# LBM-EPFL/MaD

Measured on AMD Instinct MI355X. Metric: anchor-pair x rotation correlations/sec on 256^3 map; top-k pose agreement, higher is better.
Workload: dtype i8 (correlation, exact int32 accumulate) / f64 (binning, pose scoring)

## Files before the change

### mad_amd/csrc/mad_common.h

```cpp
#pragma once

#include <hip/hip_runtime.h>

#include <cmath>
#include <cstdarg>
#include <cstdint>
#include <cstdio>
#include <cstdlib>
#include <cstring>

#include "../../include/mad_amd.h"

#define MAD_WAVE 64
#define MAD_ZLUT 1024
#define MAD_MAX_BELT 32


struct __attribute__((aligned(16))) EqspFastLds {
    float g32[MAD_MAX_Z][4];
    float z_in_lo[MAD_MAX_BELT], z_in_hi[MAD_MAX_BELT], belt_lo0[MAD_MAX_BELT], belt_inv_w[MAD_MAX_BELT];
    int belt_first[MAD_MAX_BELT], belt_count[MAD_MAX_BELT];
    unsigned char zlut[MAD_ZLUT];
    float4 belt_f[MAD_MAX_BELT];
    int2 belt_i[MAD_MAX_BELT];
// ... 19 lines not shown

struct EqspDev {
    int Z;
    int nbelt;
    double th_lo[MAD_MAX_Z];
    double th_hi[MAD_MAX_Z];
    double ph_lo[MAD_MAX_Z];
    double ph_hi[MAD_MAX_Z];
    int belt_first[MAD_MAX_Z];
    int belt_count[MAD_MAX_Z];
    double to_dom[MAD_MAX_Z][9];
    double adj_sec[MAD_MAX_Z][9];
    unsigned char zlut[MAD_ZLUT];
    float z_in_lo[MAD_MAX_BELT];
    float z_in_hi[MAD_MAX_BELT];
    float belt_lo0[MAD_MAX_BELT];
    float belt_inv_w[MAD_MAX_BELT];
    int belt_first32[MAD_MAX_BELT];
    int belt_count32[MAD_MAX_BELT];
    float g32[MAD_MAX_Z][4];
    EqspFastLds image;
    EqspTabLds tab;
    int tab_ok;
};

#ifndef MAD_EQSP_GUARD
#define MAD_EQSP_GUARD 4e-5
#endif

struct FieldDev {
    const float4 *tex;
    int nx, ny, nz;
    const unsigned *tex4;
};


struct DevBuf {
    void *p = nullptr;
    size_t cap = 0;
};

enum { MAD_T_ORIENT = 0, MAD_T_DESCRIBE, MAD_T_CORRELATE, MAD_T_PAIRS, MAD_T_POSE, MAD_T_TOPK, MAD_T_REFINE,
       MAD_T_DENSITY, MAD_T_CCC, MAD_T_SEG_PARENT, MAD_T_SEG_JUMP, MAD_T_SEG_SCAN, MAD_T_SEG_SMOOTH, MAD_T_COUNT };

#define MAD_T_RING 32
#define MAD_LANES 8
#define MAD_BRACKETS 3
#define MAD_SHARD_RING 8
#define MAD_DIST_BUFS 6
#define MAD_RES (2 * MAD_LANES)

struct TimerGroup {
    hipEvent_t start[MAD_T_RING];
    hipEvent_t stop[MAD_T_RING];
    int pending = 0;
    double total_ms = 0.0;
    int64_t launches = 0;
};

struct DensityDev {
    float *grid = nullptr;
    float4 *grad = nullptr;
    int nx = 0, ny = 0, nz = 0;
    double o[3] = {0, 0, 0};
    double vs = 0;
};
// ... 358 lines not shown
        if (i + 2 * T < n4) d4[i + 2 * T] = v2;
        if (i + 3 * T < n4) d4[i + 3 * T] = v3;
    }
    const int tail = (int)((bytes & 15) >> 2);
    if ((int)threadIdx.x < tail) ((unsigned *)lds_dst)[4 * n4 + threadIdx.x] = ((const unsigned *)src)[4 * n4 + threadIdx.x];
}

__device__ __forceinline__ int cvt_floor(float x) {
    int r;
    asm("v_cvt_flr_i32_f32 %0, %1" : "=v"(r) : "v"(x));
    return r;
}
__device__ __forceinline__ unsigned mad_u24(unsigned a, unsigned b, unsigned c) {
    unsigned r;
    asm("v_mad_u32_u24 %0, %1, %2, %3" : "=v"(r) : "v"(a), "v"(b), "v"(c));
    return r;
}
__device__ __forceinline__ int cvt_round(float x) {
    int r;
    asm("v_cvt_rpi_i32_f32 %0, %1" : "=v"(r) : "v"(x));
    return r;
}

__device__ __forceinline__ void eqsp_fast_stage(const EqspDev *t, EqspFastLds *l) { stage_lds(l, &t->image, sizeof(EqspFastLds)); }

__device__ __forceinline__ unsigned mad_tex4_encode(float x, float y, float z, float w) {
    if (!(fabsf(x) <= 3.0e38f) || !(fabsf(y) <= 3.0e38f) || !(fabsf(z) <= 3.0e38f) || !(w <= 3.0e38f)) return 0x80000000u;
    if (w < 1e-5f) return 0xC0000000u;
    const float inv = 511.0f / w;
    const int ix = min(max((int)rintf(x * inv), -511), 511), iy = min(max((int)rintf(y * inv), -511), 511), iz = min(max((int)rintf(z * inv), -511), 511);
    return ((unsigned)ix & 0x3ffu) | (((unsigned)iy & 0x3ffu) << 10) | (((unsigned)iz & 0x3ffu) << 20);
}

__device__ __forceinline__ int eqsp_tab32(const EqspTabLds *t, float x, float y, float z) {
    const int bz = min(max(cvt_floor(fmaf(z, 0.5f * MAD_TAB_ZBINS, 0.5f * MAD_TAB_ZBINS)), 0), MAD_TAB_ZBINS - 1);
    const int b = t->zbelt[bz];
    const float xr = x * __builtin_amdgcn_rcpf(fmaxf(fabsf(x) + fabsf(y), 1e-30f));
    const float u = copysignf(fmaf(xr, 0.25f * MAD_TAB_PBINS, 0.25f * MAD_TAB_PBINS), y);
    const int bp = min(max(cvt_floor(0.5f * MAD_TAB_PBINS - u), 0), MAD_TAB_PBINS - 1);
    const int zn = t->ptab[b & (MAD_TAB_BELTS - 1)][bp];
    return (b | zn) >= 255 ? -1 : zn;
}

template <class F>
__device__ __forceinline__ void eqsp_classify_lds(const EqspFastLds *t, double th, double sth, double ph, F &&f) {
    const int nb = t->nbelt;
    for (int b = 0; b < nb; b++) {
        if (ph < t->ph_hi[b] && ph > t->ph_lo[b]) {
            const int a0 = t->belt_first[b], a1 = a0 + t->belt_count[b];
            for (int a = a0; a < a1; a++) {
                const double lo = t->th_lo[a], hi = t->th_hi[a];
                if ((th < hi && th > lo) || (sth < hi && sth > lo)) f(a);
            }
            break;
        }
    }
}

__device__ __forceinline__ float approx_angle(float x, float y) {
    const float ax = fabsf(x), ay = fabsf(y);
    const float mx = fmaxf(ax, ay), mn = fminf(ax, ay);
    const float q = mn * __builtin_amdgcn_rcpf(fmaxf(mx, 1e-30f));
    const float q2 = q * q;
    float a = fmaf(q2, -0.011769974f, 0.052822195f);
    a = fmaf(q2, a, -0.116649978f);
    a = fmaf(q2, a, 0.193669885f);
// ... 78 lines not shown
```

### mad_amd/csrc/mad_ctx.hip

```cpp
#include "mad_common.h"

static char g_init_err[512] = "";
#define MAD_TWO_PI_H 6.283185307179586476925286766559

int mad_fail(mad_ctx *ctx, int code, const char *fmt, ...) {
    char *dst = ctx ? ctx->err : g_init_err;
    va_list ap;
    va_start(ap, fmt);
    vsnprintf(dst, 512, fmt, ap);
    va_end(ap);
    return code;
}

extern "C" const char *mad_last_error(const mad_ctx *ctx) { return ctx ? ctx->err : g_init_err; }

int mad_reserve(mad_ctx *ctx, DevBuf &b, size_t bytes) {
    if (bytes == 0) bytes = 16;
    if (b.cap >= bytes) return MAD_OK;
    if (b.p) {
        MAD_HIP(hipStreamSynchronize(ctx->stream));
        (void)hipFree(b.p);
        b.p = nullptr;
        b.cap = 0;
    }
// ... 305 lines not shown
        for (int a = 0; a < MAD_MAX_Z; a++) { im.th_lo[a] = h.th_lo[a]; im.th_hi[a] = h.th_hi[a]; }
        im.nbelt = h.nbelt;
        im.tier2_ok = getenv("MAD_NO_TIER2") ? 0 : 1;
        for (int a = 0; a < Z; a++) {
            im.dir[a][0] = cos(h.th_lo[a]); im.dir[a][1] = sin(h.th_lo[a]);
            im.dir[a][2] = cos(h.th_hi[a]); im.dir[a][3] = sin(h.th_hi[a]);
        }
        for (int b = 0; b < h.nbelt; b++) {
            const double m[2] = {MAD_T2_MARGIN64, MAD_T2_MARGIN32};
            for (int k = 0; k < 2; k++) {
                im.zthr[b][2 * k] = h.ph_lo[b] <= 0.0 ? 2.0 : cos(h.ph_lo[b] + m[k]);
                im.zthr[b][2 * k + 1] = h.ph_hi[b] - m[k] >= 3.14159265358979323846 ? -2.0 : cos(h.ph_hi[b] - m[k]);
            }
            if (h.belt_count[b] > 1)
                for (int a = h.belt_first[b]; a < h.belt_first[b] + h.belt_count[b]; a++)
                    if (!(h.th_hi[a] - h.th_lo[a] < 3.0) || !(h.th_hi[a] > h.th_lo[a])) im.tier2_ok = 0;
            if (b + 1 < h.nbelt && h.ph_hi[b] != h.ph_lo[b + 1]) im.tier2_ok = 0;
        }
    }
    {
        static const bool no_tab = getenv("MAD_NO_TAB") != nullptr;
        h.tab_ok = mad_eqsp_tab_build(bounds, Z, h.tab.zbelt, &h.tab.ptab[0][0]) == 1 && !no_tab ? 1 : 0;
    }
    if (to_dom) memcpy(h.to_dom, to_dom, sizeof(double) * 9 * Z);
    if (adj_sec) memcpy(h.adj_sec, adj_sec, sizeof(double) * 9 * Z);
    MAD_HIP(hipMemcpyAsync(ctx->eq[which], &h, sizeof(EqspDev), hipMemcpyHostToDevice, ctx->stream));
    MAD_HIP(hipStreamSynchronize(ctx->stream));
    ctx->eq_set[which] = true;
    return MAD_OK;
}


__global__ __launch_bounds__(256) void k_pack_field(const float *__restrict__ gx, const float *__restrict__ gy,
                                                    const float *__restrict__ gz, float4 *__restrict__ tex, unsigned *__restrict__ tex4, size_t n) {
    size_t i = (size_t)blockIdx.x * blockDim.x + threadIdx.x;
    const size_t step = (size_t)gridDim.x * blockDim.x;
    for (; i < n; i += step) {
        const float x = gx[i], y = gy[i], z = gz[i];
        const float s = __fadd_rn(__fadd_rn(__fmul_rn(x, x), __fmul_rn(y, y)), __fmul_rn(z, z));
        const float w = sqrtf(s);
        tex[i] = make_float4(x, y, z, w);
        tex4[i] = mad_tex4_encode(x, y, z, w);
    }
}

int mad_field_alloc(mad_ctx *ctx, int slot, int nx, int ny, int nz, size_t *n_out) {
    if (slot < 0 || slot >= MAD_MAX_FIELDS) return mad_fail(ctx, MAD_EINVAL, "field slot %d out of range", slot);
    if (nx < 2 || ny < 2 || nz < 2) return mad_fail(ctx, MAD_EINVAL, "field dims %dx%dx%d", nx, ny, nz);
    const size_t n = (size_t)nx * ny * nz;
    if (n >= ((size_t)1 << 32) || (size_t)nx * ny >= ((size_t)1 << 24) || nz >= (1 << 24))
        return mad_fail(ctx, MAD_EINVAL, "field of %dx%dx%d texels: more than 2^32 texels or 2^24 per x-y plane", nx, ny, nz);
    if (ctx->field_mem[slot]) {
        MAD_HIP(hipStreamSynchronize(ctx->stream));
        (void)hipFree(ctx->field_mem[slot]);
        ctx->field_mem[slot] = nullptr;
        ctx->fields[slot] = FieldDev{nullptr, 0, 0, 0};
    }
    hipError_t e = hipMalloc(&ctx->field_mem[slot], n * (sizeof(float4) + sizeof(unsigned)));
    if (e != hipSuccess) {
        ctx->field_mem[slot] = nullptr;
        return mad_fail(ctx, MAD_ENOMEM, "field of %zu texels: %s", n, hipGetErrorString(e));
    }
    ctx->fields[slot] = FieldDev{(const float4 *)ctx->field_mem[slot], nx, ny, nz, (const unsigned *)((const float4 *)ctx->field_mem[slot] + n)};
    *n_out = n;
    return MAD_OK;
}

extern "C" int mad_upload_field_device(mad_ctx *ctx, int slot, const float *g3, int nx, int ny, int nz) {
    if (!ctx || !g3) return MAD_EINVAL;
    size_t n = 0;
    MAD_TRY(mad_field_alloc(ctx, slot, nx, ny, nz, &n));
    const int blocks = (int)std::min<size_t>(mad_ceil_div((int64_t)n, 256), (size_t)ctx->n_cu * 16);
    hipLaunchKernelGGL(k_pack_field, dim3(blocks), dim3(256), 0, ctx->stream, g3, g3 + n, g3 + 2 * n,
                       (float4 *)ctx->field_mem[slot], (unsigned *)((float4 *)ctx->field_mem[slot] + n), n);
    MAD_HIP(hipGetLastError());
    MAD_HIP(hipStreamSynchronize(ctx->stream));
    return MAD_OK;
}

extern "C" int mad_upload_field(mad_ctx *ctx, int slot, const float *gx, const float *gy, const float *gz, int nx,
                                int ny, int nz) {
    if (!ctx || !gx || !gy || !gz) return MAD_EINVAL;
    const size_t n = (size_t)nx * ny * nz;
    float *stage = nullptr;
    hipError_t e = hipMalloc((void **)&stage, 3 * n * sizeof(float));
    if (e != hipSuccess) return mad_fail(ctx, MAD_ENOMEM, "field staging: %s", hipGetErrorString(e));
    int rc = MAD_OK;
    if (hipMemcpyAsync(stage, gx, n * sizeof(float), hipMemcpyHostToDevice, ctx->stream) != hipSuccess ||
        hipMemcpyAsync(stage + n, gy, n * sizeof(float), hipMemcpyHostToDevice, ctx->stream) != hipSuccess ||
        hipMemcpyAsync(stage + 2 * n, gz, n * sizeof(float), hipMemcpyHostToDevice, ctx->stream) != hipSuccess)
        rc = mad_fail(ctx, MAD_EHIP, "field upload failed");
    if (rc == MAD_OK) rc = mad_upload_field_device(ctx, slot, stage, nx, ny, nz);
    (void)hipStreamSynchronize(ctx->stream);
    (void)hipFree(stage);
    return rc;
}

extern "C" int mad_free_field(mad_ctx *ctx, int slot) {
    if (!ctx || slot < 0 || slot >= MAD_MAX_FIELDS) return MAD_EINVAL;
    if (ctx->field_mem[slot]) {
        MAD_HIP(hipStreamSynchronize(ctx->stream));
        (void)hipFree(ctx->field_mem[slot]);
    }
    ctx->field_mem[slot] = nullptr;
    ctx->fields[slot] = FieldDev{nullptr, 0, 0, 0};
    return MAD_OK;
}

extern "C" int mad_field_download(mad_ctx *ctx, int slot, float *tex_xyzw, uint32_t *tex4) {
    if (!ctx) return MAD_EINVAL;
    if (slot < 0 || slot >= MAD_MAX_FIELDS || !ctx->field_mem[slot]) return mad_fail(ctx, MAD_EINVAL, "mad_field_download: slot %d is empty or out of range", slot);
    const FieldDev &f = ctx->fields[slot];
    const size_t n = (size_t)f.nx * f.ny * f.nz;
    MAD_HIP(hipStreamSynchronize(ctx->stream));
    if (tex_xyzw) MAD_HIP(hipMemcpyAsync(tex_xyzw, f.tex, n * sizeof(float4), hipMemcpyDeviceToHost, ctx->stream));
    if (tex4) MAD_HIP(hipMemcpyAsync(tex4, f.tex4, n * sizeof(unsigned), hipMemcpyDeviceToHost, ctx->stream));
    MAD_HIP(hipStreamSynchronize(ctx->stream));
    return MAD_OK;
}


__global__ __launch_bounds__(256) void k_zero_words(uint4 *__restrict__ p, size_t n16) {
    for (size_t i = (size_t)blockIdx.x * blockDim.x + threadIdx.x; i < n16; i += (size_t)gridDim.x * blockDim.x) p[i] = make_uint4(0, 0, 0, 0);
}

__global__ __launch_bounds__(256) void k_copy_words(uint4 *__restrict__ dst, const uint4 *__restrict__ src, size_t n16) {
    for (size_t i = (size_t)blockIdx.x * blockDim.x + threadIdx.x; i < n16; i += (size_t)gridDim.x * blockDim.x) dst[i] = src[i];
}

void mad_zero_words(mad_ctx *ctx, void *p, size_t bytes) {
    const size_t n16 = (bytes + 15) / 16;
    hipLaunchKernelGGL(k_zero_words, dim3((unsigned)std::min<size_t>((n16 + 255) / 256, 1024)), dim3(256), 0, ctx->stream, (uint4 *)p, n16);
}

__global__ __launch_bounds__(256) void k_zero_words3(uint4 *__restrict__ p, size_t n16, uint4 *__restrict__ q, size_t m16, uint4 *__restrict__ r,
                                                     size_t l16) {
    for (size_t i = (size_t)blockIdx.x * blockDim.x + threadIdx.x; i < n16 + m16 + l16; i += (size_t)gridDim.x * blockDim.x) {
        if (i < n16) p[i] = make_uint4(0, 0, 0, 0);
        else if (i < n16 + m16) q[i - n16] = make_uint4(0, 0, 0, 0);
        else r[i - n16 - m16] = make_uint4(0, 0, 0, 0);
    }
}

void mad_zero_words3(mad_ctx *ctx, void *p, size_t bytes_p, void *q, size_t bytes_q, void *r, size_t bytes_r) {
    const size_t n16 = (bytes_p + 15) / 16, m16 = (bytes_q + 15) / 16, l16 = (bytes_r + 15) / 16;
    hipLaunchKernelGGL(k_zero_words3, dim3((unsigned)std::min<size_t>((n16 + m16 + l16 + 255) / 256, 1024)), dim3(256), 0, ctx->stream, (uint4 *)p,
                       n16, (uint4 *)q, m16, (uint4 *)r, l16);
}

void mad_copy_words(mad_ctx *ctx, void *dst, const void *src, size_t bytes) {
// ... 194 lines not shown
```

### mad_amd/csrc/mad_orient.hip

```cpp
#include <type_traits>

#include "mad_common.h"

#ifndef ORI_THREADS
#define ORI_THREADS 512
#endif
#define ORI_MAX_FAN 64
#define ORI_QUEUE 512
#define ORI_MAX_MAIN 8


static int ensure_mask(mad_ctx *ctx, int r) {
    if (ctx->mask_r == r) return MAD_OK;
    const int B = 2 * r + 1;
    int8_t *h = (int8_t *)malloc((size_t)B * B * B * 4);
    int n = 0;
    for (int i = -r; i <= r; i++)
        for (int j = -r; j <= r; j++)
            for (int k = -r; k <= r; k++)
                if (sqrt((double)(i * i + j * j + k * k)) <= r * 1.05) {
                    h[4 * n] = (int8_t)i; h[4 * n + 1] = (int8_t)j; h[4 * n + 2] = (int8_t)k; h[4 * n + 3] = 0;
                    n++;
                }
    if (ctx->mask_off) {
// ... 716 lines not shown
    const EqspDev *eq;
    int16_t *dsc;
    int8_t *dsc8;
    double *norm;
    int32_t *rsum;
};

__device__ __forceinline__ int describe_exact(const EqspFastLds *eq, float4 t, const double *R) {
    float gx = t.x, gy = t.y, gz = t.z;
    if (t.w > 1e-12f) { gx = __fdiv_rn(gx, t.w); gy = __fdiv_rn(gy, t.w); gz = __fdiv_rn(gz, t.w); }
    const double g0 = gx, g1 = gy, g2 = gz;
    const double rx = g0 * R[0] + g1 * R[1] + g2 * R[2];
    const double ry = g0 * R[3] + g1 * R[4] + g2 * R[5];
    const double rz = g0 * R[6] + g1 * R[7] + g2 * R[8];
    int zone = 0;
    classify_exact64(eq, eq, rx, ry, rz, [&](int zn) { zone = zn; });
    return zone;
}

__device__ __forceinline__ bool lattice_voxel_exact(double l0, double l1, double l2, const double *inv, double c0, double c1, double c2,
                                                    const FieldDev &F, int *v0, int *v1, int *v2) {
    const double p0 = (l0 * inv[0] + l1 * inv[1] + l2 * inv[2]) + c0;
    const double p1 = (l0 * inv[3] + l1 * inv[4] + l2 * inv[5]) + c1;
    const double p2 = (l0 * inv[6] + l1 * inv[7] + l2 * inv[8]) + c2;
    if (!(p0 >= 0.0) || !(p0 <= (double)(F.nx - 1)) || !(p1 >= 0.0) || !(p1 <= (double)(F.ny - 1)) || !(p2 >= 0.0) ||
        !(p2 <= (double)(F.nz - 1)))
        return false;
    int a0i = min((int)floor(p0), F.nx - 2), a1i = min((int)floor(p1), F.ny - 2), a2i = min((int)floor(p2), F.nz - 2);
    *v0 = (p0 - (double)a0i <= 0.5) ? a0i : a0i + 1;
    *v1 = (p1 - (double)a1i <= 0.5) ? a1i : a1i + 1;
    *v2 = (p2 - (double)a2i <= 0.5) ? a2i : a2i + 1;
    return true;
}
__device__ __forceinline__ unsigned lattice_index_exact(double l0, double l1, double l2, const double *inv, double c0, double c1, double c2,
                                                        const FieldDev &F, bool *oob) {
    int a0i, a1i, a2i;
    if (!lattice_voxel_exact(l0, l1, l2, inv, c0, c1, c2, F, &a0i, &a1i, &a2i)) {
        *oob = true;
        return 0;
    }
    return (unsigned)(((size_t)a0i * F.ny + a1i) * F.nz + a2i);
}

template <int S, int NSUB> __device__ __forceinline__ int sub_blk(int x) {
    if (NSUB == 64) return x / (S / 4);
    if (NSUB == 27) return x < S / 3 ? 0 : (x < 2 * S / 3 ? 1 : 2);
    if (NSUB == 8) return x < S / 2 ? 0 : 1;
    return 0;
}
template <int S, int NSUB> __device__ __forceinline__ int sub_of_jk(int j, int k) {
    if (NSUB == 64) return sub_blk<S, NSUB>(j) * 16 + sub_blk<S, NSUB>(k);
    if (NSUB == 27) return sub_blk<S, NSUB>(j) * 9 + sub_blk<S, NSUB>(k);
    if (NSUB == 8) return sub_blk<S, NSUB>(j) * 2 + (1 - sub_blk<S, NSUB>(k));
    return 0;
}
template <int S, int NSUB> __device__ __forceinline__ int sub_of_i(int i) {
    if (NSUB == 64) return sub_blk<S, NSUB>(i) * 4;
    if (NSUB == 27) return sub_blk<S, NSUB>(i) * 3;
    if (NSUB == 8) return sub_blk<S, NSUB>(i) * 4;
    return 0;
}

#define DSC_CHUNK 8
#ifndef DSC_PASSES
#define DSC_PASSES 1
#endif
#ifndef DSC_OCC
#define DSC_OCC 4
#endif
#define DSC_QUEUE_TAB 768
#ifdef MAD_PROBE_STAMPS
__device__ long long dsc_stamps[16384 * 8];
__device__ int dsc_open[16384];
// ... 60 lines not shown
    const int D = NSUB * Z;
    for (int i = tid; i < D; i += NT) hist[i] = 0;
    const int32_t *const p_perm = A.row_perm, *const p_anchor = A.row_anchor, *const p_coords = A.anc_coords, *const p_octave = A.anc_octave;
    const double *const p_R = A.row_R, *const p_Rinv = A.row_Rinv;
    const int uni_octave = A.uniform_octave;
    auto chain_record = [=](int64_t w, int *rec) {
        const int r = p_perm ? p_perm[w] : (int)w;
        const int an = p_anchor ? p_anchor[r] : r;
        rec[0] = r;
        rec[1] = p_coords[3 * an]; rec[2] = p_coords[3 * an + 1]; rec[3] = p_coords[3 * an + 2];
        rec[4] = p_octave ? p_octave[an] : uni_octave;
        double *inv = (double *)(rec + 8);
        if (p_Rinv) {
            for (int i = 0; i < 9; i++) inv[i] = p_Rinv[9 * (int64_t)r + i];
        } else {
            double m[9];
            mad_mat3_inv(p_R + 9 * (int64_t)r, m);
            for (int i = 0; i < 9; i++) inv[i] = m[i];
        }
    };
    const int *const recs = (const int *)A.row_rec;
    if (recs) {
        if (tid < 32) s_rec[tid] = recs[work * MAD_ROWREC_WORDS + tid];
    } else if (tid == 0) chain_record(work, s_rec);
    if (tid == 0) { s_oob = 0; s_nq = 0; }
    __syncthreads();
    const int64_t row = __builtin_amdgcn_readfirstlane(s_rec[0]);
    const int oct = __builtin_amdgcn_readfirstlane(s_rec[4]);
    const double *const sInv = (const double *)&s_rec[8];
    FieldDev F;
    F.tex = oct == 1 ? F1.tex : F0.tex; F.nx = oct == 1 ? F1.nx : F0.nx; F.ny = oct == 1 ? F1.ny : F0.ny; F.nz = oct == 1 ? F1.nz : F0.nz;
    F.tex4 = oct == 1 ? F1.tex4 : F0.tex4;
#ifdef DSC_TEX_AUX
    const __amdgpu_buffer_rsrc_t tex_rsrc = __builtin_amdgcn_make_buffer_rsrc((void *)F.tex4, 0, F.nx * F.ny * F.nz * 4, 0x00020000);
#define DSC_TEX4(at) ((unsigned)__builtin_amdgcn_raw_buffer_load_b32(tex_rsrc, (int)((at) * 4u), 0, DSC_TEX_AUX))
#else
#define DSC_TEX4(at) (F.tex4[at])
#endif
    const double *Rrow = A.row_R + 9 * row;
    DSC_STAMP(1);

    const int ic0 = __builtin_amdgcn_readfirstlane(s_rec[1]), ic1 = __builtin_amdgcn_readfirstlane(s_rec[2]),
              ic2 = __builtin_amdgcn_readfirstlane(s_rec[3]);
    const float h0 = (float)sInv[0], h1 = (float)sInv[1], h2 = (float)sInv[2], h3 = (float)sInv[3], h4 = (float)sInv[4], h5 = (float)sInv[5],
                h6 = (float)sInv[6], h7 = (float)sInv[7], h8 = (float)sInv[8];
    const int j = tid / S, k = tid % S;
    const bool active = tid < S * S;
    const float lbf = oct == 0 ? (float)(-2 * A.r + 1) : (float)-A.r + 0.5f, lsf = oct == 0 ? 2.0f : 1.0f;
    auto exact_index = [&](int i, bool *left) -> unsigned {
        float lb = lbf, ls = lsf;
        asm volatile("" : "+v"(lb), "+v"(ls));
        const double lbase = (double)lb, lstep = (double)ls;
        return lattice_index_exact(lbase + lstep * i, lbase + lstep * j, lbase + lstep * k, sInv, (double)ic0, (double)ic1, (double)ic2, F, left);
    };
    const int reach = (int)(1.7320508 * fabs((double)lbf)) + 2;
    const bool interior = ic0 - reach >= 1 && ic0 + reach <= F.nx - 2 && ic1 - reach >= 1 && ic1 + reach <= F.ny - 2 &&
                          ic2 - reach >= 1 && ic2 + reach <= F.nz - 2;
    constexpr int NP = S > 16 ? (S % DSC_CHUNK == 0 ? S / DSC_CHUNK : 2) : ((S % (DSC_CHUNK * DSC_PASSES) == 0) ? DSC_PASSES : 1);
    constexpr int PS = S / NP;
    static_assert(S % NP == 0 && PS <= 32, "a pass's samples are one bit each of `unsure` / `undecided`");
#define UBIT(i) (TAB ? PS - 1 - (i) : (i))
    bool oob = false;
    if (active) {
        const float m1 = lbf + lsf * (float)j, m2 = lbf + lsf * (float)k;
        const float b0 = fmaf(m1, h1, m2 * h2), b1 = fmaf(m1, h4, m2 * h5), b2 = fmaf(m1, h7, m2 * h8);
        const int sub_jk = sub_of_jk<S, NSUB>(j, k);
        const int sjk16 = sub_jk * 16;
#pragma unroll
        for (int pass = 0; pass < NP; pass++) {
            float4 t[TAB ? 1 : PS];
            unsigned q4[TAB ? PS : 1], qi[TAB ? PS : 1];
            unsigned unsure = 0;
            auto guess = [&](auto border) {
                constexpr bool CARRY = TAB && !decltype(border)::value;
                const float fc0 = (float)ic0, fc1 = (float)ic1, fc2 = (float)ic2;
                const float lim0 = (float)(F.nx - 1) - 1e-3f, lim1 = (float)(F.ny - 1) - 1e-3f, lim2 = (float)(F.nz - 1) - 1e-3f;
#pragma unroll
                for (int i = 0; i < PS; i++) {
                    const float m0 = lbf + lsf * (float)(pass * PS + i);
                    const float a0 = fmaf(m0, h0, b0), a1 = fmaf(m0, h3, b1), a2 = fmaf(m0, h6, b2);
                    const float fr0 = __builtin_amdgcn_fractf(a0), fr1 = __builtin_amdgcn_fractf(a1), fr2 = __builtin_amdgcn_fractf(a2);
                    const float tie = fminf(fminf(fabsf(fr0 - 0.5f), fabsf(fr1 - 0.5f)), fabsf(fr2 - 0.5f));
                    bool safe = tie > 2e-4f;
                    if (CARRY) asm("v_cmp_nlt_f32 vcc, %1, %2\n\tv_addc_co_u32 %0, vcc, %0, %0, vcc" : "+v"(unsure) : "s"(2e-4f), "v"(tie) : "vcc");
                    int n0 = ic0 + cvt_round(a0), n1 = ic1 + cvt_round(a1), n2 = ic2 + cvt_round(a2);
                    if (decltype(border)::value) {
                        const float q0 = a0 + fc0, q1 = a1 + fc1, q2 = a2 + fc2;
                        safe &= (q0 > 1e-3f) & (q0 < lim0) & (q1 > 1e-3f) & (q1 < lim1) & (q2 > 1e-3f) & (q2 < lim2);
                        n0 = min(max(n0, 0), F.nx - 1); n1 = min(max(n1, 0), F.ny - 1); n2 = min(max(n2, 0), F.nz - 1);
                    }
                    const unsigned at = mad_u24(mad_u24((unsigned)n0, (unsigned)F.ny, (unsigned)n1), (unsigned)F.nz, (unsigned)n2);
                    if (TAB) { qi[i] = at; q4[i] = DSC_TEX4(at); }
                    else t[i] = F.tex[at];
                    if (!CARRY) unsure |= safe ? 0u : (1u << UBIT(i));
                }
            };
            if (interior) guess(std::false_type()); else guess(std::true_type());
            DSC_STAMP(2);
            if (unsure) {
#pragma unroll
                for (int i = 0; i < PS; i++)
                    if (unsure & (1u << UBIT(i))) {
                        const unsigned at = exact_index(pass * PS + i, &oob);
                        if (TAB) { qi[i] = at; q4[i] = DSC_TEX4(at); }
                        else t[i] = F.tex[at];
                    }
            }
            unsigned undecided = 0;
            const float zs = TAB ? (1.0f / 511.0f) : 1.0f;
            const float f0 = (float)Rrow[0], f1 = (float)Rrow[1], f2 = (float)Rrow[2], f3 = (float)Rrow[3], f4 = (float)Rrow[4], f5 = (float)Rrow[5],
                        f6 = (float)Rrow[6] * zs, f7 = (float)Rrow[7] * zs, f8 = (float)Rrow[8] * zs;
#pragma unroll
            for (int i0 = 0; i0 < PS; i0 += DSC_CHUNK) {
                int zone[DSC_CHUNK];
                unsigned any_flag = 0;
#pragma unroll
                for (int u = 0; u < DSC_CHUNK; u++) {
                    if (i0 + u >= PS) { zone[u] = -2; continue; }
                    if (TAB) {
                        const unsigned q = q4[i0 + u];
                        const float gx = (float)(int)__builtin_amdgcn_sbfe(q, 0, 10), gy = (float)(int)__builtin_amdgcn_sbfe(q, 10, 10),
                                    gz = (float)(int)__builtin_amdgcn_sbfe(q, 20, 10);
                        const float rx = fmaf(gz, f2, fmaf(gy, f1, gx * f0));
                        const float ry = fmaf(gz, f5, fmaf(gy, f4, gx * f3));
                        const float rz = fmaf(gz, f8, fmaf(gy, f7, gx * f6));
                        const int zn = eqsp_tab32((const EqspTabLds *)&tab, rx, ry, rz);
                        zone[u] = zn;
                        any_flag |= q;
                        continue;
                    }
                    const float4 tx = t[i0 + u];
                    const float inv = __builtin_amdgcn_rcpf(fmaxf(tx.w, 1e-30f));
                    const float gx = tx.x * inv, gy = tx.y * inv, gz = tx.z * inv;
                    const float rx = fmaf(gz, f2, fmaf(gy, f1, gx * f0));
                    const float ry = fmaf(gz, f5, fmaf(gy, f4, gx * f3));
                    const float rz = fmaf(gz, f8, fmaf(gy, f7, gx * f6));
// ... 33 lines not shown
                            off++;
                        }
                }
            } else if (undecided) {
#pragma unroll
                for (int i = 0; i < PS; i++)
                    if (undecided & (1u << i)) {
                        const int slot = atomicAdd(&s_nq, 1);
                        if (slot < QCAP) { qv[slot] = t[i]; qsub[slot] = sub_jk + sub_of_i<S, NSUB>(pass * PS + i); }
                    }
            }
        }
    }
    DSC_STAMP(4);
    if (oob) s_oob = 1;
    __syncthreads();
    DSC_STAMP(5);
    DSC_NOTE_OPEN(s_nq);
    const bool dead = s_oob != 0;
    if (dead) {
        for (int i = tid; i < D; i += NT) A.dsc[row * D + i] = 0;
        if (A.dsc8) {
            for (int i = tid; i < D; i += NT) A.dsc8[row * D + i] = WIDE ? (int8_t)-MAD_WIDE_C : 0;
            if (tid == 0) A.norm[row] = 0.0;
            if (WIDE && tid == 0) A.rsum[row] = MAD_WIDE_BIAS(0, D);
        }
    } else if (s_nq > QCAP) {
        __syncthreads();
        for (int i = tid; i < D; i += NT) hist[i] = 0;
        __syncthreads();
        if (active)
            for (int i = 0; i < S; i++) {
                bool none = false;
                const float4 tx = F.tex[exact_index(i, &none)];
                if (tx.w < 1e-5f) continue;
                atomicAdd(&hist[(sub_of_jk<S, NSUB>(j, k) + sub_of_i<S, NSUB>(i)) * Z + describe_exact(exactp, tx, Rrow)], 1);
            }
    } else if (TAB) {
        const int nq = s_nq;
        const float f0 = (float)Rrow[0], f1 = (float)Rrow[1], f2 = (float)Rrow[2], f3 = (float)Rrow[3], f4 = (float)Rrow[4], f5 = (float)Rrow[5],
                    f6 = (float)Rrow[6], f7 = (float)Rrow[7], f8 = (float)Rrow[8];
        for (int e = tid; e < nq; e += NT) {
            const float4 tx = F.tex[qidx[e]];
            if (tx.w < 1e-5f) continue;
            const float inv = __builtin_amdgcn_rcpf(fmaxf(tx.w, 1e-30f));
            const float gx = tx.x * inv, gy = tx.y * inv, gz = tx.z * inv;
            int zn = eqsp_fast32(fastp, fmaf(gz, f2, fmaf(gy, f1, gx * f0)), fmaf(gz, f5, fmaf(gy, f4, gx * f3)), fmaf(gz, f8, fmaf(gy, f7, gx * f6)));
            if (zn < 0) zn = describe_exact(exactp, tx, Rrow);
            atomicAdd(&hist[(int)qsub16[e] * Z + zn], 1);
        }
    } else {
        const int nq = s_nq;
        for (int qi = tid; qi < nq; qi += NT) atomicAdd(&hist[qsub[qi] * Z + describe_exact(exactp, qv[qi], Rrow)], 1);
    }
    __syncthreads();
    DSC_STAMP(6);
    int ss = 0;
    int sv = 0;
    for (int i = tid; i < D; i += NT) {
        const int v = hist[i];
        if (dead) continue;
        A.dsc[row * D + i] = (int16_t)v;
        if (A.dsc8) A.dsc8[row * D + i] = (int8_t)(WIDE ? v - MAD_WIDE_C : v);
        ss += v * v;
        if (WIDE) sv += v;
    }
    if (A.dsc8 && !dead) {
        ss = wave_sum_i32(ss);
        if (lane_id() == 0) s_part[tid >> 6] = ss;
        if (WIDE) {
            sv = wave_sum_i32(sv);
            if (lane_id() == 0) s_sum[tid >> 6] = sv;
        }
        __syncthreads();
        if (tid == 0) {
            int tot = 0;
// ... 117 lines not shown
```

### mad_amd/csrc/mad_space.hip

```cpp
#include <algorithm>
#include <cstring>
#include <vector>

#include "mad_common.h"

namespace {

struct Dims {
    int n[3];
    __host__ __device__ size_t count() const { return (size_t)n[0] * n[1] * n[2]; }
};

__device__ __forceinline__ int reflect_idx(int i, int n) {
    if (n == 1) return 0;
    const int p = 2 * n;
    i %= p;
    if (i < 0) i += p;
    return i < n ? i : p - 1 - i;
}

template <typename T>
__global__ __launch_bounds__(256) void k_pad(const T *__restrict__ src, Dims s, int pad, T *__restrict__ dst, Dims d) {
    const size_t total = d.count();
    for (size_t i = (size_t)blockIdx.x * blockDim.x + threadIdx.x; i < total; i += (size_t)gridDim.x * blockDim.x) {
// ... 79 lines not shown
        if (w1) out1[i] = (Tout)a1;
    }
}

template <typename T>
__global__ __launch_bounds__(256) void k_log_gauss(const T *__restrict__ s01, const T *__restrict__ u01, const T *__restrict__ t01, Dims d,
                                                   int R, const double *__restrict__ g0, const double *__restrict__ g2, double sig2,
                                                   T *__restrict__ gauss, T *__restrict__ logv) {
    const size_t total = d.count();
    const int n = d.n[2];
    for (size_t i = (size_t)blockIdx.x * blockDim.x + threadIdx.x; i < total; i += (size_t)gridDim.x * blockDim.x) {
        const int pos = (int)(i % n);
        const size_t base = i - pos;
        const double cs = (double)s01[i], cu = (double)u01[i], ct = (double)t01[i];
        double a0 = cs * g0[R], a1 = cu * g0[R], a2 = ct * g2[R], ag = ct * g0[R];
        for (int jj = -R; jj < 0; jj++) {
            const size_t il = base + reflect_idx(pos + jj, n), ir = base + reflect_idx(pos - jj, n);
            const double ps = (double)s01[il] + (double)s01[ir], pu = (double)u01[il] + (double)u01[ir], pt = (double)t01[il] + (double)t01[ir];
            a0 += ps * g0[R + jj];
            a1 += pu * g0[R + jj];
            a2 += pt * g2[R + jj];
            ag += pt * g0[R + jj];
        }
        gauss[i] = (T)ag;
        T l = (T)a0;
        l = l + (T)a1;
        l = l + (T)a2;
        l = (-l) * (T)sig2;
        logv[i] = (l < (T)0) ? (T)0 : l;
    }
}

template <typename T>
__global__ __launch_bounds__(256) void k_grad_tex(const T *__restrict__ g, Dims d, float4 *__restrict__ tex, unsigned *__restrict__ tex4) {
    const size_t total = d.count();
    const size_t sx = (size_t)d.n[1] * d.n[2], sy = (size_t)d.n[2];
    for (size_t i = (size_t)blockIdx.x * blockDim.x + threadIdx.x; i < total; i += (size_t)gridDim.x * blockDim.x) {
        const int z = (int)(i % d.n[2]), y = (int)((i / d.n[2]) % d.n[1]), x = (int)(i / sx);
        T gx, gy, gz;
        if (x == 0) gx = g[i + sx] - g[i]; else if (x == d.n[0] - 1) gx = g[i] - g[i - sx]; else gx = (g[i + sx] - g[i - sx]) / (T)2;
        if (y == 0) gy = g[i + sy] - g[i]; else if (y == d.n[1] - 1) gy = g[i] - g[i - sy]; else gy = (g[i + sy] - g[i - sy]) / (T)2;
        if (z == 0) gz = g[i + 1] - g[i]; else if (z == d.n[2] - 1) gz = g[i] - g[i - 1]; else gz = (g[i + 1] - g[i - 1]) / (T)2;
        const float fx = (float)gx, fy = (float)gy, fz = (float)gz;
        const float s = __fadd_rn(__fadd_rn(__fmul_rn(fx, fx), __fmul_rn(fy, fy)), __fmul_rn(fz, fz));
        const float w = sqrtf(s);
        tex[i] = make_float4(fx, fy, fz, w);
        tex4[i] = mad_tex4_encode(fx, fy, fz, w);
    }
}

template <typename Tin, typename Tout>
__global__ __launch_bounds__(256) void k_convert(const Tin *__restrict__ in, Tout *__restrict__ out, size_t n) {
    for (size_t i = (size_t)blockIdx.x * blockDim.x + threadIdx.x; i < n; i += (size_t)gridDim.x * blockDim.x) out[i] = (Tout)in[i];
}

template <typename T>
__global__ __launch_bounds__(256) void k_peaks(const T *__restrict__ v, Dims d, double thr, int border, int64_t *__restrict__ out_idx,
                                               double *__restrict__ out_val, int32_t *__restrict__ count, int cap) {
    const size_t total = d.count();
    const size_t sx = (size_t)d.n[1] * d.n[2], sy = (size_t)d.n[2];
    const T thr_t = (T)thr;
    for (size_t i = (size_t)blockIdx.x * blockDim.x + threadIdx.x; i < total; i += (size_t)gridDim.x * blockDim.x) {
        const int z = (int)(i % d.n[2]), y = (int)((i / d.n[2]) % d.n[1]), x = (int)(i / sx);
        if (x < border || y < border || z < border || x >= d.n[0] - border || y >= d.n[1] - border || z >= d.n[2] - border) continue;
        const T c = v[i];
        if (!(c > thr_t)) continue;
        bool is_max = !(c < (T)0);
        for (int dx = -1; dx <= 1 && is_max; dx++) {
            for (int dy = -1; dy <= 1 && is_max; dy++) {
                for (int dz = -1; dz <= 1; dz++) {
                    const int xx = x + dx, yy = y + dy, zz = z + dz;
                    T o = (T)0;
                    if (xx >= 0 && xx < d.n[0] && yy >= 0 && yy < d.n[1] && zz >= 0 && zz < d.n[2]) o = v[(size_t)xx * sx + (size_t)yy * sy + zz];
                    if (o > c) { is_max = false; break; }
                }
            }
        }
        if (!is_max) continue;
        const int slot = atomicAdd(count, 1);
        if (slot < cap) { out_idx[slot] = (int64_t)i; out_val[slot] = (double)c; }
// ... 180 lines not shown
}

extern "C" int mad_space_create(mad_ctx *ctx, mad_space **out) {
    if (!ctx || !out) return MAD_EINVAL;
    *out = new mad_space();
    return MAD_OK;
}

extern "C" void mad_space_destroy(mad_ctx *ctx, mad_space *s) {
    if (!s) return;
    if (ctx) (void)hipStreamSynchronize(ctx->stream);
    space_release(s);
    delete s;
}

template <typename T>
static int build_octave(mad_ctx *ctx, Octave &O, int R, const double *d_g0, const double *d_g2, double sig2, int slot) {
    Arena A;
    const size_t n = O.d.count(), bytes = n * sizeof(T);
    const unsigned nb = blocks_for(ctx, n);
    T *grid = (T *)O.grid;
    T *t0 = (T *)A.get(bytes), *s0 = (T *)A.get(bytes), *t01 = (T *)A.get(bytes), *s01 = (T *)A.get(bytes), *u01 = (T *)A.get(bytes);
    if (!t0 || !s0 || !t01 || !s01 || !u01) return mad_fail(ctx, MAD_ENOMEM, "mad_space_build: %zu bytes of filter temporaries", 5 * bytes);
    if (hipMalloc(&O.gauss, bytes) != hipSuccess || hipMalloc(&O.logv, bytes) != hipSuccess)
        return mad_fail(ctx, MAD_ENOMEM, "mad_space_build: %zu bytes of volumes", 2 * bytes);
    hipLaunchKernelGGL((k_filter_axis<T, T>), dim3(nb), dim3(256), 0, ctx->stream, grid, O.d, 0, R, d_g0, d_g2, t0, s0);
    hipLaunchKernelGGL((k_filter_axis<T, T>), dim3(nb), dim3(256), 0, ctx->stream, t0, O.d, 1, R, d_g0, d_g2, t01, u01);
    hipLaunchKernelGGL((k_filter_axis<T, T>), dim3(nb), dim3(256), 0, ctx->stream, s0, O.d, 1, R, d_g0, (const double *)nullptr, s01, (T *)nullptr);
    hipLaunchKernelGGL((k_log_gauss<T>), dim3(nb), dim3(256), 0, ctx->stream, s01, u01, t01, O.d, R, d_g0, d_g2, sig2, (T *)O.gauss, (T *)O.logv);
    MAD_HIP(hipGetLastError());
    if (slot >= 0) {
        size_t cnt = 0;
        MAD_TRY(mad_field_alloc(ctx, slot, O.d.n[0], O.d.n[1], O.d.n[2], &cnt));
        hipLaunchKernelGGL((k_grad_tex<T>), dim3(nb), dim3(256), 0, ctx->stream, (const T *)O.gauss, O.d, (float4 *)ctx->field_mem[slot],
                           (unsigned *)((float4 *)ctx->field_mem[slot] + cnt));
        MAD_HIP(hipGetLastError());
    }
    MAD_HIP(hipStreamSynchronize(ctx->stream));
    return MAD_OK;
}

template <typename T>
static int build_all(mad_ctx *ctx, mad_space *s, const T *h_grid, int nx, int ny, int nz, int pad, int oct_mode, const double *g0,
                     const double *g2, int R, double sig2, const double *pre, int pre_R, const double *const *lu,
                     const double *const *ev_w, const int32_t *const *ev_i, int slot_up, int slot_base) {
    Arena A;
    const Dims src{{nx, ny, nz}};
    const Dims b{{nx + 2 * pad, ny + 2 * pad, nz + 2 * pad}};
    double *d_g0 = (double *)A.get((2 * R + 1) * 8), *d_g2 = (double *)A.get((2 * R + 1) * 8), *d_pre = (double *)A.get((2 * pre_R + 1) * 8);
    T *d_src = (T *)A.get(src.count() * sizeof(T));
    if (!d_g0 || !d_g2 || !d_pre || !d_src) return mad_fail(ctx, MAD_ENOMEM, "mad_space_build: staging");
    MAD_HIP(hipMemcpyAsync(d_g0, g0, (2 * R + 1) * 8, hipMemcpyHostToDevice, ctx->stream));
    MAD_HIP(hipMemcpyAsync(d_g2, g2, (2 * R + 1) * 8, hipMemcpyHostToDevice, ctx->stream));
    if (pre_R > 0) MAD_HIP(hipMemcpyAsync(d_pre, pre, (2 * pre_R + 1) * 8, hipMemcpyHostToDevice, ctx->stream));
    MAD_HIP(hipMemcpyAsync(d_src, h_grid, src.count() * sizeof(T), hipMemcpyHostToDevice, ctx->stream));
    T *base = nullptr;
    if (hipMalloc((void **)&base, b.count() * sizeof(T)) != hipSuccess) return mad_fail(ctx, MAD_ENOMEM, "mad_space_build: base volume");
    hipLaunchKernelGGL((k_pad<T>), dim3(blocks_for(ctx, b.count())), dim3(256), 0, ctx->stream, (const T *)d_src, src, pad, base, b);
    MAD_HIP(hipGetLastError());

    int n_oct = 0;
    if (oct_mode & 2) {
        Dims cur = b;
        const void *in = base;
        bool in_is_T = true;
        double *vol = nullptr;
        for (int a = 0; a < 3; a++) {
            const int n = cur.n[a];
// ... 214 lines not shown
```

Before: 111.3 billion.

## Store packed tex4 gradient field in 4x4x2 bricks for gather locality

Reorders the 4-byte packed gradient texture into bricks of 4x4x2 voxels (32 words, 128 bytes) instead of linear x-y-z order. Producers, the descriptor sampling path and host readback are all updated to use the brick index, and a reverse mapping recovers the linear voxel for float4 lookups. The goal is for rotated-lattice gathers in the describe kernel to touch fewer cache lines. In exchange there is extra index arithmetic per sample, padded allocation with zero fill, and a host-side unshuffle on readback.

```diff
diff --git a/mad_amd/csrc/mad_common.h b/mad_amd/csrc/mad_common.h
--- a/mad_amd/csrc/mad_common.h
+++ b/mad_amd/csrc/mad_common.h
@@ -75,6 +75,10 @@
     const float4 *tex;
     int nx, ny, nz;
     const unsigned *tex4;
+    __host__ __device__ unsigned nbx() const { return ((unsigned)nx + 3u) >> 2; }
+    __host__ __device__ unsigned nby() const { return ((unsigned)ny + 3u) >> 2; }
+    __host__ __device__ unsigned nbz() const { return ((unsigned)nz + 1u) >> 1; }
+    __host__ __device__ size_t tex4_words() const { return (size_t)32 * nbx() * nby() * nbz(); }
 };
 
 
@@ -499,6 +503,22 @@
     return ((unsigned)ix & 0x3ffu) | (((unsigned)iy & 0x3ffu) << 10) | (((unsigned)iz & 0x3ffu) << 20);
 }
 
+__host__ __device__ __forceinline__ unsigned mad_tex4_index(const FieldDev &F, unsigned x, unsigned y, unsigned z) {
+#ifdef __HIP_DEVICE_COMPILE__
+    const unsigned brick = mad_u24(mad_u24(x >> 2, F.nby(), y >> 2), F.nbz(), z >> 1);
+#else
+    const unsigned brick = ((x >> 2) * F.nby() + (y >> 2)) * F.nbz() + (z >> 1);
+#endif
+    return (brick << 5) | ((x & 3u) << 3) | ((y & 3u) << 1) | (z & 1u);
+}
+__host__ __device__ __forceinline__ unsigned mad_tex4_voxel(const FieldDev &F, unsigned at) {
+    const unsigned brick = at >> 5, nby = F.nby(), nbz = F.nbz();
+    const unsigned t = brick / nbz, bz = brick - t * nbz;
+    const unsigned bx = t / nby, by = t - bx * nby;
+    const unsigned x = (bx << 2) | ((at >> 3) & 3u), y = (by << 2) | ((at >> 1) & 3u), z = (bz << 1) | (at & 1u);
+    return (x * (unsigned)F.ny + y) * (unsigned)F.nz + z;
+}
+
 __device__ __forceinline__ int eqsp_tab32(const EqspTabLds *t, float x, float y, float z) {
     const int bz = min(max(cvt_floor(fmaf(z, 0.5f * MAD_TAB_ZBINS, 0.5f * MAD_TAB_ZBINS)), 0), MAD_TAB_ZBINS - 1);
     const int b = t->zbelt[bz];
diff --git a/mad_amd/csrc/mad_ctx.hip b/mad_amd/csrc/mad_ctx.hip
--- a/mad_amd/csrc/mad_ctx.hip
+++ b/mad_amd/csrc/mad_ctx.hip
@@ -361,7 +361,10 @@
 
 
 __global__ __launch_bounds__(256) void k_pack_field(const float *__restrict__ gx, const float *__restrict__ gy,
-                                                    const float *__restrict__ gz, float4 *__restrict__ tex, unsigned *__restrict__ tex4, size_t n) {
+                                                    const float *__restrict__ gz, FieldDev F, size_t n) {
+    float4 *const tex = (float4 *)F.tex;
+    unsigned *const tex4 = (unsigned *)F.tex4;
+    const size_t sx = (size_t)F.ny * F.nz;
     size_t i = (size_t)blockIdx.x * blockDim.x + threadIdx.x;
     const size_t step = (size_t)gridDim.x * blockDim.x;
     for (; i < n; i += step) {
@@ -369,7 +372,8 @@
         const float s = __fadd_rn(__fadd_rn(__fmul_rn(x, x), __fmul_rn(y, y)), __fmul_rn(z, z));
         const float w = sqrtf(s);
         tex[i] = make_float4(x, y, z, w);
-        tex4[i] = mad_tex4_encode(x, y, z, w);
+        const unsigned vx = (unsigned)(i / sx), vyz = (unsigned)(i - (size_t)vx * sx);
+        tex4[mad_tex4_index(F, vx, vyz / (unsigned)F.nz, vyz % (unsigned)F.nz)] = mad_tex4_encode(x, y, z, w);
     }
 }
 
@@ -379,18 +383,25 @@
     const size_t n = (size_t)nx * ny * nz;
     if (n >= ((size_t)1 << 32) || (size_t)nx * ny >= ((size_t)1 << 24) || nz >= (1 << 24))
         return mad_fail(ctx, MAD_EINVAL, "field of %dx%dx%d texels: more than 2^32 texels or 2^24 per x-y plane", nx, ny, nz);
+    FieldDev geo{nullptr, nx, ny, nz, nullptr};
+    const size_t n4 = geo.tex4_words();
+    if (n4 >= ((size_t)1 << 32) || (size_t)geo.nbx() * geo.nby() >= ((size_t)1 << 24) || geo.nbz() >= (1u << 24))
+        return mad_fail(ctx, MAD_EINVAL, "field of %dx%dx%d texels: more than 2^32 4-byte texels in bricks of 4x4x2", nx, ny, nz);
     if (ctx->field_mem[slot]) {
         MAD_HIP(hipStreamSynchronize(ctx->stream));
         (void)hipFree(ctx->field_mem[slot]);
         ctx->field_mem[slot] = nullptr;
         ctx->fields[slot] = FieldDev{nullptr, 0, 0, 0};
     }
-    hipError_t e = hipMalloc(&ctx->field_mem[slot], n * (sizeof(float4) + sizeof(unsigned)));
+    const size_t off4 = (n * sizeof(float4) + 127) / 128 * 128;
+    hipError_t e = hipMalloc(&ctx->field_mem[slot], off4 + n4 * sizeof(unsigned));
     if (e != hipSuccess) {
         ctx->field_mem[slot] = nullptr;
         return mad_fail(ctx, MAD_ENOMEM, "field of %zu texels: %s", n, hipGetErrorString(e));
     }
-    ctx->fields[slot] = FieldDev{(const float4 *)ctx->field_mem[slot], nx, ny, nz, (const unsigned *)((const float4 *)ctx->field_mem[slot] + n)};
+    ctx->fields[slot] = FieldDev{(const float4 *)ctx->field_mem[slot], nx, ny, nz, (const unsigned *)((const char *)ctx->field_mem[slot] + off4)};
+    mad_zero_words(ctx, (void *)ctx->fields[slot].tex4, n4 * sizeof(unsigned));
+    MAD_HIP(hipGetLastError());
     *n_out = n;
     return MAD_OK;
 }
@@ -400,8 +411,7 @@
     size_t n = 0;
     MAD_TRY(mad_field_alloc(ctx, slot, nx, ny, nz, &n));
     const int blocks = (int)std::min<size_t>(mad_ceil_div((int64_t)n, 256), (size_t)ctx->n_cu * 16);
-    hipLaunchKernelGGL(k_pack_field, dim3(blocks), dim3(256), 0, ctx->stream, g3, g3 + n, g3 + 2 * n,
-                       (float4 *)ctx->field_mem[slot], (unsigned *)((float4 *)ctx->field_mem[slot] + n), n);
+    hipLaunchKernelGGL(k_pack_field, dim3(blocks), dim3(256), 0, ctx->stream, g3, g3 + n, g3 + 2 * n, ctx->fields[slot], n);
     MAD_HIP(hipGetLastError());
     MAD_HIP(hipStreamSynchronize(ctx->stream));
     return MAD_OK;
@@ -443,8 +453,18 @@
     const size_t n = (size_t)f.nx * f.ny * f.nz;
     MAD_HIP(hipStreamSynchronize(ctx->stream));
     if (tex_xyzw) MAD_HIP(hipMemcpyAsync(tex_xyzw, f.tex, n * sizeof(float4), hipMemcpyDeviceToHost, ctx->stream));
-    if (tex4) MAD_HIP(hipMemcpyAsync(tex4, f.tex4, n * sizeof(unsigned), hipMemcpyDeviceToHost, ctx->stream));
+    std::vector<unsigned> bricks;
+    if (tex4) {
+        bricks.resize(f.tex4_words());
+        MAD_HIP(hipMemcpyAsync(bricks.data(), f.tex4, bricks.size() * sizeof(unsigned), hipMemcpyDeviceToHost, ctx->stream));
+    }
     MAD_HIP(hipStreamSynchronize(ctx->stream));
+    if (tex4) {
+        size_t i = 0;
+        for (int x = 0; x < f.nx; x++)
+            for (int y = 0; y < f.ny; y++)
+                for (int z = 0; z < f.nz; z++) tex4[i++] = bricks[mad_tex4_index(f, (unsigned)x, (unsigned)y, (unsigned)z)];
+    }
     return MAD_OK;
 }
 
diff --git a/mad_amd/csrc/mad_orient.hip b/mad_amd/csrc/mad_orient.hip
--- a/mad_amd/csrc/mad_orient.hip
+++ b/mad_amd/csrc/mad_orient.hip
@@ -772,6 +772,7 @@
     *v2 = (p2 - (double)a2i <= 0.5) ? a2i : a2i + 1;
     return true;
 }
+template <bool BRICK>
 __device__ __forceinline__ unsigned lattice_index_exact(double l0, double l1, double l2, const double *inv, double c0, double c1, double c2,
                                                         const FieldDev &F, bool *oob) {
     int a0i, a1i, a2i;
@@ -779,6 +780,7 @@
         *oob = true;
         return 0;
     }
+    if (BRICK) return mad_tex4_index(F, (unsigned)a0i, (unsigned)a1i, (unsigned)a2i);
     return (unsigned)(((size_t)a0i * F.ny + a1i) * F.nz + a2i);
 }
 
@@ -905,7 +907,7 @@
     F.tex = oct == 1 ? F1.tex : F0.tex; F.nx = oct == 1 ? F1.nx : F0.nx; F.ny = oct == 1 ? F1.ny : F0.ny; F.nz = oct == 1 ? F1.nz : F0.nz;
     F.tex4 = oct == 1 ? F1.tex4 : F0.tex4;
 #ifdef DSC_TEX_AUX
-    const __amdgpu_buffer_rsrc_t tex_rsrc = __builtin_amdgcn_make_buffer_rsrc((void *)F.tex4, 0, F.nx * F.ny * F.nz * 4, 0x00020000);
+    const __amdgpu_buffer_rsrc_t tex_rsrc = __builtin_amdgcn_make_buffer_rsrc((void *)F.tex4, 0, (int)(F.tex4_words() * 4), 0x00020000);
 #define DSC_TEX4(at) ((unsigned)__builtin_amdgcn_raw_buffer_load_b32(tex_rsrc, (int)((at) * 4u), 0, DSC_TEX_AUX))
 #else
 #define DSC_TEX4(at) (F.tex4[at])
@@ -920,11 +922,11 @@
     const int j = tid / S, k = tid % S;
     const bool active = tid < S * S;
     const float lbf = oct == 0 ? (float)(-2 * A.r + 1) : (float)-A.r + 0.5f, lsf = oct == 0 ? 2.0f : 1.0f;
-    auto exact_index = [&](int i, bool *left) -> unsigned {
+    auto exact_index = [&](int i, bool *left, auto brick) -> unsigned {
         float lb = lbf, ls = lsf;
         asm volatile("" : "+v"(lb), "+v"(ls));
         const double lbase = (double)lb, lstep = (double)ls;
-        return lattice_index_exact(lbase + lstep * i, lbase + lstep * j, lbase + lstep * k, sInv, (double)ic0, (double)ic1, (double)ic2, F, left);
+        return lattice_index_exact<decltype(brick)::value>(lbase + lstep * i, lbase + lstep * j, lbase + lstep * k, sInv, (double)ic0, (double)ic1, (double)ic2, F, left);
     };
     const int reach = (int)(1.7320508 * fabs((double)lbf)) + 2;
     const bool interior = ic0 - reach >= 1 && ic0 + reach <= F.nx - 2 && ic1 - reach >= 1 && ic1 + reach <= F.ny - 2 &&
@@ -962,7 +964,8 @@
                         safe &= (q0 > 1e-3f) & (q0 < lim0) & (q1 > 1e-3f) & (q1 < lim1) & (q2 > 1e-3f) & (q2 < lim2);
                         n0 = min(max(n0, 0), F.nx - 1); n1 = min(max(n1, 0), F.ny - 1); n2 = min(max(n2, 0), F.nz - 1);
                     }
-                    const unsigned at = mad_u24(mad_u24((unsigned)n0, (unsigned)F.ny, (unsigned)n1), (unsigned)F.nz, (unsigned)n2);
+                    const unsigned at = TAB ? mad_tex4_index(F, (unsigned)n0, (unsigned)n1, (unsigned)n2)
+                                            : mad_u24(mad_u24((unsigned)n0, (unsigned)F.ny, (unsigned)n1), (unsigned)F.nz, (unsigned)n2);
                     if (TAB) { qi[i] = at; q4[i] = DSC_TEX4(at); }
                     else t[i] = F.tex[at];
                     if (!CARRY) unsure |= safe ? 0u : (1u << UBIT(i));
@@ -974,7 +977,7 @@
 #pragma unroll
                 for (int i = 0; i < PS; i++)
                     if (unsure & (1u << UBIT(i))) {
-                        const unsigned at = exact_index(pass * PS + i, &oob);
+                        const unsigned at = exact_index(pass * PS + i, &oob, std::integral_constant<bool, TAB>());
                         if (TAB) { qi[i] = at; q4[i] = DSC_TEX4(at); }
                         else t[i] = F.tex[at];
                     }
@@ -1074,7 +1077,7 @@
         if (active)
             for (int i = 0; i < S; i++) {
                 bool none = false;
-                const float4 tx = F.tex[exact_index(i, &none)];
+                const float4 tx = F.tex[exact_index(i, &none, std::false_type())];
                 if (tx.w < 1e-5f) continue;
                 atomicAdd(&hist[(sub_of_jk<S, NSUB>(j, k) + sub_of_i<S, NSUB>(i)) * Z + describe_exact(exactp, tx, Rrow)], 1);
             }
@@ -1083,7 +1086,7 @@
         const float f0 = (float)Rrow[0], f1 = (float)Rrow[1], f2 = (float)Rrow[2], f3 = (float)Rrow[3], f4 = (float)Rrow[4], f5 = (float)Rrow[5],
                     f6 = (float)Rrow[6], f7 = (float)Rrow[7], f8 = (float)Rrow[8];
         for (int e = tid; e < nq; e += NT) {
-            const float4 tx = F.tex[qidx[e]];
+            const float4 tx = F.tex[mad_tex4_voxel(F, qidx[e])];
             if (tx.w < 1e-5f) continue;
             const float inv = __builtin_amdgcn_rcpf(fmaxf(tx.w, 1e-30f));
             const float gx = tx.x * inv, gy = tx.y * inv, gz = tx.z * inv;
diff --git a/mad_amd/csrc/mad_space.hip b/mad_amd/csrc/mad_space.hip
--- a/mad_amd/csrc/mad_space.hip
+++ b/mad_amd/csrc/mad_space.hip
@@ -135,7 +135,9 @@
 }
 
 template <typename T>
-__global__ __launch_bounds__(256) void k_grad_tex(const T *__restrict__ g, Dims d, float4 *__restrict__ tex, unsigned *__restrict__ tex4) {
+__global__ __launch_bounds__(256) void k_grad_tex(const T *__restrict__ g, Dims d, FieldDev F) {
+    float4 *const tex = (float4 *)F.tex;
+    unsigned *const tex4 = (unsigned *)F.tex4;
     const size_t total = d.count();
     const size_t sx = (size_t)d.n[1] * d.n[2], sy = (size_t)d.n[2];
     for (size_t i = (size_t)blockIdx.x * blockDim.x + threadIdx.x; i < total; i += (size_t)gridDim.x * blockDim.x) {
@@ -148,7 +150,7 @@
         const float s = __fadd_rn(__fadd_rn(__fmul_rn(fx, fx), __fmul_rn(fy, fy)), __fmul_rn(fz, fz));
         const float w = sqrtf(s);
         tex[i] = make_float4(fx, fy, fz, w);
-        tex4[i] = mad_tex4_encode(fx, fy, fz, w);
+        tex4[mad_tex4_index(F, (unsigned)x, (unsigned)y, (unsigned)z)] = mad_tex4_encode(fx, fy, fz, w);
     }
 }
 
@@ -395,8 +397,7 @@
     if (slot >= 0) {
         size_t cnt = 0;
         MAD_TRY(mad_field_alloc(ctx, slot, O.d.n[0], O.d.n[1], O.d.n[2], &cnt));
-        hipLaunchKernelGGL((k_grad_tex<T>), dim3(nb), dim3(256), 0, ctx->stream, (const T *)O.gauss, O.d, (float4 *)ctx->field_mem[slot],
-                           (unsigned *)((float4 *)ctx->field_mem[slot] + cnt));
+        hipLaunchKernelGGL((k_grad_tex<T>), dim3(nb), dim3(256), 0, ctx->stream, (const T *)O.gauss, O.d, ctx->fields[slot]);
         MAD_HIP(hipGetLastError());
     }
     MAD_HIP(hipStreamSynchronize(ctx->stream));
```

New measurement: 120.7 billion, median of 6. +8.4%, better.
